# hoyso48/AudioTokenization

Hardware: AMD Instinct MI355X
Metric: audio-sec encoded/sec/GPU (24 kHz mono, 10 s clips) + VQ index bit-exactness (higher is better)
Workload: dtype f32-emulated (x6: 3xbf16, 24-bit operands); 1 GPU; config2: batch=64 x 10 s 24 kHz clips per GPU, encode+VQ (extract_indices path), BigCodec 'default' model, random weights; global_batch=64, clip_samples=240000, parallelism=dp1

## Files before the change

### audiotokenization_amd/csrc/conv1d_x6_kernel.h

```cpp
#pragma once
#include <type_traits>

#include "bc_common.h"
#include "bc_internal.h"
#include "conv_epilogue.h"
#include "x6_common.h"

namespace bc {

struct X6NoMid {};

template <int MT, int NT, int WM, int WN, int P, bool PW, int TPS = 1, bool DB = false, bool B4 = false>
__global__ void __launch_bounds__(64 * WM * WN, (WM * WN == 16 ? 1 : (NT == 1 ? 4 : 2))) conv1d_x6_kernel(ConvArgs a) {
  constexpr int BM = 16 * MT * WM;
  constexpr int BN = 16 * NT * WN;
  constexpr int QA = WM * MT;
  constexpr int NW = WM * WN;
  static_assert(NW == 8 || NW == 16, "512- or 1024-thread workgroups");
  constexpr int NCG = NW / 8;
  constexpr int CI = ((PW ? BN / 32 : X6_MAXCOL_ITERS) + NCG - 1) / NCG;
  constexpr int NQI = 4 * NW;
  constexpr int IT4 = PW ? (BN / 4 + NQI - 1) / NQI : ((32 * X6_MAXCOL_ITERS + 6) / 4 + NQI - 1) / NQI;
  constexpr int NBL = B4 ? 2 * IT4 : 2 * CI;
  extern __shared__ __attribute__((aligned(16))) unsigned char smem_x6[];
// ... 811 lines not shown
          compute(step & 1, 0, tp, mid);
        } else {
          if (step + 1 < nsteps && !BC_ABL(a.dbg, 1)) issue_a(step + 1, (step + 1) & 1);
          if (tp == 0 && c + 1 < a.nchunks && !BC_ABL(a.dbg, 2)) {
            dma_issue_order();
            stage_load(c + 1);
          }
          if (prio) __builtin_amdgcn_s_setprio(1);
#pragma unroll
          for (int tt = 0; tt < TPS; ++tt) {
            const int tap = tp * TPS + tt;
            if (TPS == 1 || tap < K) compute(step & 1, tt, tap, nomid);
          }
        }
        if (prio) __builtin_amdgcn_s_setprio(0);
        if constexpr (DB) {
          if (c + 1 < a.nchunks) {
            if (P == 2 && tp == 1) stage_max((c + 1) & 1);
            if (tp == DB_STORE) {
              if constexpr (P == 2) {
                const float sn = bmax_scale((c + 1) & 1);
                xn = sn < xs ? sn : xs;
              }
              if (!BC_ABL(a.dbg, 4)) stage_store(Bs + ((c + 1) & 1) * P * bplane, xn, c + 1);
            }
          }
        } else if (tp == kst - 1 && c + 1 < a.nchunks) {
          if constexpr (P == 2) stage_max((c + 1) & 1);
          lds_barrier();
          if constexpr (P == 2) h3_next_scale((c + 1) & 1);
          if (!BC_ABL(a.dbg, 4)) stage_store(Bs, xs, c + 1);
        }
        if (tp == 0 && kst > 1 && c + 1 < a.nchunks)
          wait_vmcnt<NBL>();
        else
          asm volatile("s_waitcnt vmcnt(0)" ::: "memory");
        lds_barrier();
      }
      if constexpr (DB && P == 2) rescale_to(xn);
    }
  }

  fin(acc, b, m0, n0, wm, wn, lane, xs);
}

inline constexpr X6Tile kX6Tiles[] = {
    {4, 4, 2, 4},
    {4, 2, 2, 4},
    {4, 2, 4, 2},
    {2, 2, 4, 2},
    {6, 2, 1, 8},
    {4, 2, 1, 8},
    {3, 2, 1, 8},
    {2, 2, 1, 8},
    {1, 2, 1, 8},
    {6, 1, 1, 8},
    {4, 1, 1, 8},
    {3, 1, 1, 8},
    {2, 1, 1, 8},
    {1, 1, 1, 8},
    {6, 2, 2, 4},
    {6, 1, 2, 4},
    {3, 1, 2, 4},
    {4, 1, 2, 4},
    {8, 2, 2, 4},
    {4, 4, 4, 2},
    {6, 4, 2, 4},
    {8, 4, 2, 4},
    {6, 2, 2, 8},
    {3, 2, 2, 4},
    {3, 4, 1, 8},
};
constexpr int X6_NT = sizeof(kX6Tiles) / sizeof(kX6Tiles[0]);

inline size_t x6_lds(const X6Tile& t, int ncol, int planes, int s, int tps = 1, int bbufs = 1) {
  const size_t bplane = (size_t)((ncol * x6_pitch(s) + 15) / 16 * 16);
  return bbufs * planes * bplane + 2 * tps * planes * (size_t)t.WM * t.MT * 1024;
}

inline int x6_tps() {
  static const int v = [] {
    const char* e = getenv("BC_X6_TPS");
    return e && atoi(e) == 1 ? 1 : 2;
  }();
  return v;
}

inline bool x6_pw_on() {
  static const bool v = [] {
    const char* e = getenv("BC_X6_PW");
    return !e || atoi(e) != 0;
  }();
  return v;
}

inline bool x6_db_on() {
  static const bool v = [] {
    const char* e = getenv("BC_X6_DB");
    return !e || atoi(e) != 0;
  }();
  return v;
}

inline bool x6_tps4_on() {
  static const bool v = [] {
    const char* e = getenv("BC_X6_TPS4");
    return !e || atoi(e) != 0;
  }();
  return v;
}

inline bool x6_b4_on() {
  static const bool v = [] {
    const char* e = getenv("BC_X6_B4");
    return !e || atoi(e) != 0;
  }();
  return v;
}

struct X6Variant {
  bool pw;
  int tps;
  bool db;
  size_t lds;
  bool b4;
};
inline X6Variant x6_variant_base(const X6Tile& t, int P, int K, int s, int d) {
  const int ncol = x6_ncol(t, K, s, d);
  const size_t budget = t.NT > 1 ? 160 * 1024 : 80 * 1024;
  auto fits = [&](int tps, int bb) { return x6_lds(t, ncol, P, s, tps, bb) <= budget; };
  if (K == 1 && ncol == x6_BN(t) && x6_pw_on()) return {true, 1, false, x6_lds(t, ncol, P, s), false};
  const int min_kst = P == 2 ? 3 : 2;
  const bool db = x6_db_on() && P <= 2 && t.NT > 1;
  const bool tps2 = P <= 2 && K > 1 && x6_tps() == 2;
  if (P == 1 && t.WM * t.WN == 16 && db && tps2 && x6_tps4_on() && (K + 3) / 4 >= min_kst && fits(4, 2))
    return {false, 4, true, x6_lds(t, ncol, P, s, 4, 2), false};
  if (db && tps2 && (K + 1) / 2 >= min_kst && fits(2, 2)) return {false, 2, true, x6_lds(t, ncol, P, s, 2, 2), false};
  if (tps2 && fits(2, 1)) return {false, 2, false, x6_lds(t, ncol, P, s, 2), false};
  if (db && K >= min_kst && fits(1, 2)) return {false, 1, true, x6_lds(t, ncol, P, s, 1, 2), false};
  return {false, 1, false, x6_lds(t, ncol, P, s), false};
}
inline X6Variant x6_variant(const X6Tile& t, int P, int K, int s, int d, int ps = 0) {
  X6Variant v = x6_variant_base(t, P, K, s, d);
  const bool pw_tile = t.WM * t.WN == 16 || (t.MT == 6 && t.NT == 2 && t.WM == 2 && t.WN == 4);
  v.b4 = s == 1 && ps == 0 && x6_b4_on() && (v.pw ? pw_tile : t.WM * t.WN == 16);
  return v;
}
inline int x6_prio() {
  static const int v = [] {
    const char* e = getenv("BC_X6_PRIO");
    return e ? atoi(e) : 0;
  }();
  return v;
}
inline bool x6_b4_fits(const ConvArgs& a) {
  return a.ps == 0 && a.s == 1 && a.Tin % 4 == 0 && a.xbs % 4 == 0 && ((unsigned long long)a.x & 15) == 0;
}

template <int MT, int NT, int WM, int WN, int P>
static int launch_x6(ConvArgs& a, int B, hipStream_t st) {
  constexpr int BM = 16 * MT * WM, BN = 16 * NT * WN, NTHR = 64 * WM * WN;
  const X6Tile t{MT, NT, WM, WN};
  const int ncol = x6_ncol(t, a.K, a.s, a.d);
  if (ncol > 32 * X6_MAXCOL_ITERS) return BC_ERR_UNSUPPORTED;
  a.ntm = (a.Cout + BM - 1) / BM;
  a.ntn = (a.Nout + BN - 1) / BN;
  a.nchunks = (a.Cin + X6_BKC - 1) / X6_BKC;
  a.win = ncol;
  a.bpitch = x6_pitch(a.s);
  a.bstage = (ncol * a.bpitch + 15) / 16 * 16;
  const long long nwg = (long long)a.ntm * a.ntn * B;
  if (nwg <= 0) return BC_OK;
  if (nwg > 0x7fffffffLL) return BC_ERR_ARG;
  if ((long long)(a.ps ? a.cin0 : a.Cin) * a.Tin * 4 > 0x7fffffffLL) return BC_ERR_UNSUPPORTED;
  a.nwg = (int)nwg;
  a.wsc = P == 2 ? reinterpret_cast<const float*>(reinterpret_cast<const unsigned char*>(a.w) +
                                                  (long long)a.ntm * a.nchunks * a.K * P * t.WM * t.MT * 1024)
                 : nullptr;
  const size_t lds = x6_lds(t, ncol, P, a.s);
  if (lds > 160 * 1024) return BC_ERR_UNSUPPORTED;
  const X6Variant v = x6_variant(t, P, a.K, a.s, a.d, a.ps);
  a.prio = x6_prio();
  constexpr int T2 = P <= 2 ? 2 : 1;
  constexpr bool D2 = P <= 2;
  if constexpr (WM * WN == 16) {
    if (v.b4 && x6_b4_fits(a)) {
      constexpr int T4 = P == 1 ? 4 : P == 2 ? 2 : 1;
      constexpr bool D4 = P == 1;
      if (!v.pw && v.tps == T4 && v.db == D4) {
        hipLaunchKernelGGL((conv1d_x6_kernel<MT, NT, WM, WN, P, false, T4, D4, true>), dim3(a.nwg), dim3(NTHR), v.lds,
                           st, a);
        BC_CHECK_LAUNCH();
        return BC_OK;
      }
    }
  }
  if constexpr (P == 1 && WM * WN == 16) {
    if (v.tps == 4) {
      hipLaunchKernelGGL((conv1d_x6_kernel<MT, NT, WM, WN, P, false, 4, true>), dim3(a.nwg), dim3(NTHR), v.lds, st, a);
      BC_CHECK_LAUNCH();
      return BC_OK;
    }
  }
  if constexpr (WM * WN == 16 || (MT == 6 && NT == 2 && WM == 2 && WN == 4)) {
    if (v.pw && v.b4 && x6_b4_fits(a)) {
      hipLaunchKernelGGL((conv1d_x6_kernel<MT, NT, WM, WN, P, true, 1, false, true>), dim3(a.nwg), dim3(NTHR), v.lds, st, a);
      BC_CHECK_LAUNCH();
      return BC_OK;
    }
  }
  if (v.pw)
    hipLaunchKernelGGL((conv1d_x6_kernel<MT, NT, WM, WN, P, true>), dim3(a.nwg), dim3(NTHR), v.lds, st, a);
  else if (v.db && v.tps == 2)
    hipLaunchKernelGGL((conv1d_x6_kernel<MT, NT, WM, WN, P, false, T2, D2>), dim3(a.nwg), dim3(NTHR), v.lds, st, a);
  else if (v.db)
    hipLaunchKernelGGL((conv1d_x6_kernel<MT, NT, WM, WN, P, false, 1, D2>), dim3(a.nwg), dim3(NTHR), v.lds, st, a);
  else if (v.tps == 2)
    hipLaunchKernelGGL((conv1d_x6_kernel<MT, NT, WM, WN, P, false, T2>), dim3(a.nwg), dim3(NTHR), v.lds, st, a);
  else
    hipLaunchKernelGGL((conv1d_x6_kernel<MT, NT, WM, WN, P, false>), dim3(a.nwg), dim3(NTHR), v.lds, st, a);
  BC_CHECK_LAUNCH();
  return BC_OK;
}

template <int P>
static int launch_x6_w16(ConvArgs& a, int B, hipStream_t st) {
  return launch_x6<6, 2, 2, 8, P>(a, B, st);
}

template <int P>
int x6_launch_tile(ConvArgs& a, int B, int tile, hipStream_t st);

#define BC_X6_TILE_SWITCH(P)                                       \
  switch (tile) {                                                  \
    case 0: return launch_x6<4, 4, 2, 4, P>(a, B, st);             \
    case 1: return launch_x6<4, 2, 2, 4, P>(a, B, st);             \
    case 2: return launch_x6<4, 2, 4, 2, P>(a, B, st);             \
    case 3: return launch_x6<2, 2, 4, 2, P>(a, B, st);             \
    case 4: return launch_x6<6, 2, 1, 8, P>(a, B, st);             \
    case 5: return launch_x6<4, 2, 1, 8, P>(a, B, st);             \
    case 6: return launch_x6<3, 2, 1, 8, P>(a, B, st);             \
    case 7: return launch_x6<2, 2, 1, 8, P>(a, B, st);             \
    case 8: return launch_x6<1, 2, 1, 8, P>(a, B, st);             \
    case 9: return launch_x6<6, 1, 1, 8, P>(a, B, st);             \
    case 10: return launch_x6<4, 1, 1, 8, P>(a, B, st);            \
    case 11: return launch_x6<3, 1, 1, 8, P>(a, B, st);            \
    case 12: return launch_x6<2, 1, 1, 8, P>(a, B, st);            \
    case 13: return launch_x6<1, 1, 1, 8, P>(a, B, st);            \
    case 14: return launch_x6<6, 2, 2, 4, P>(a, B, st);            \
    case 15: return launch_x6<6, 1, 2, 4, P>(a, B, st);            \
    case 16: return launch_x6<3, 1, 2, 4, P>(a, B, st);            \
    case 17: return launch_x6<4, 1, 2, 4, P>(a, B, st);            \
    case 18: return launch_x6<8, 2, 2, 4, P>(a, B, st);            \
    case 19: return launch_x6<4, 4, 4, 2, P>(a, B, st);            \
    case 20: return launch_x6<6, 4, 2, 4, P>(a, B, st);            \
    case 21: return launch_x6<8, 4, 2, 4, P>(a, B, st);            \
    case 22: return launch_x6_w16<P>(a, B, st);                    \
    case 23:                                                       \
    case 24: return BC_ERR_UNSUPPORTED;                            \
  }                                                                \
  return BC_ERR_ARG;

}
```

### audiotokenization_amd/csrc/resunit_x6.hip

```cpp
#include <cstdio>
#include <cstdlib>

#include "bc_common.h"
#include "bc_internal.h"
#include "conv_epilogue.h"
#include "x6_common.h"

namespace bc {

constexpr int RU_MAX_DIL = 9;

struct RUExtra {
  const float* w1;
  const float* s2a;
  const float* s2b;
  int hplane;
  int nck1;
  int dbg;
  const float* isa;
  const float* isb;
};

__device__ __forceinline__ int hs_off(int n, int g) { return n * 64 + 16 * (g ^ ((n >> 2) & 3)); }

constexpr int ru_min_waves(int MT, int NT, int WM, int P) {
  return (NT == 1 || (MT == 3 && NT == 2 && WM == 2)) ? 4 : 2;
}
constexpr int ru_launch_waves(int MT, int NT, int WM, int WN, int P) {
  return WM * WN == 16 ? 1 : ru_min_waves(MT, NT, WM, P);
}
constexpr int ru_npw(int NW, int QA, int NTT) {
  int n = NW / QA < NTT ? NW / QA : NTT;
  while (n > 1 && NTT % n) --n;
  return n;
}

template <int MT, int NT, int WM, int WN, int P, int TPS = 1>
__global__ void __launch_bounds__(64 * WM * WN, ru_launch_waves(MT, NT, WM, WN, P)) resunit_x6_kernel(ConvArgs a, ConvArgs e, RUExtra r) {
  static_assert(P >= 1 && P <= 3, "bf16, h3 or x6 operands");
  typedef typename FragType<P>::type frag_t;
  constexpr int NW = WM * WN;
  static_assert(NW == 8 || NW == 16, "512- or 1024-thread workgroups");
  constexpr int NTHR = 64 * NW;
  constexpr int NCG = NW / 8;
  __shared__ unsigned smax[2][NW];
  constexpr int BN = 16 * NT * WN;
  constexpr int QA = WM * MT;
  constexpr int CI = ((BN + 6 * RU_MAX_DIL + 31) / 32 + NCG - 1) / NCG;
  constexpr int NTT = NT * WN;
  static_assert(QA <= NW, "one m-tile per wave in phase 2");
  constexpr int NPW = ru_npw(NW, QA, NTT);
  constexpr int NTW = NTT / NPW;
  static_assert(NTT % NPW == 0, "n-tile groups");
  constexpr int KC1 = (16 * QA + X6_BKC - 1) / X6_BKC;
  extern __shared__ __attribute__((aligned(16))) unsigned char smem_ru[];

  const int ncol = a.win;
  const int bplane = a.bstage;
  unsigned char* Bs = smem_ru;
  unsigned char* As = smem_ru + P * bplane;
  auto bgrp = [](int col, int g) { return col * 64 + 16 * (g ^ ((col >> 1) & 3)); };
  unsigned char* Hs = smem_ru;

  const int wg = xcd_remap(blockIdx.x, a.nwg);
  const int nt_idx = wg % a.ntn;
  const int b = wg / a.ntn;
  const int n0 = nt_idx * BN;

  const int tid = threadIdx.x;
  const int lane = tid & 63;
  const int wave = __builtin_amdgcn_readfirstlane(tid >> 6);
  const int wm = wave % WM;
  const int wn = wave / WM;

  const unsigned long long xb_u = (unsigned long long)(a.x + (long long)b * a.xbs);
  const unsigned xb_lo = __builtin_amdgcn_readfirstlane((unsigned)xb_u);
  const unsigned xb_hi = __builtin_amdgcn_readfirstlane((unsigned)(xb_u >> 32));
  const int xbytes = __builtin_amdgcn_readfirstlane(a.Cin * a.Tin * 4);
  const __amdgpu_buffer_rsrc_t xr = __builtin_amdgcn_make_buffer_rsrc(
      (void*)(((unsigned long long)xb_hi << 32) | xb_lo), 0, xbytes, 0x00020000);
  const int in0 = n0 - a.pl;

  const int K = a.K;
  const int kst = (K + TPS - 1) / TPS;
  const int nsteps = a.nchunks * kst;
  const int a_pieces = P * QA;

  auto issue_a = [&](const float* w, int step, int buf) {
    const int c = step / kst, t0 = (step - c * kst) * TPS;
    const int n = (K - t0 < TPS ? K - t0 : TPS) * a_pieces;
    const unsigned char* src = reinterpret_cast<const unsigned char*>(w) + (long long)(c * K + t0) * (a_pieces * 1024);
    unsigned char* dst = As + buf * (TPS * a_pieces * 1024);
    if (!BC_DOK(c < a.nchunks && t0 * a_pieces + n <= K * a_pieces)) return;
    for (int q = wave; q < n; q += NW)
      __builtin_amdgcn_global_load_lds((const void*)(src + q * 1024 + lane * 16), (lds_void_t)(dst + q * 1024),
                                       16, 0, 0);
  };

  const int bp = (tid >> 5) & 15;
  const int bcl = tid & 31;
  const int bcg = tid >> 9;
  auto bcol = [&](int i) { return bcl + 32 * (i * NCG + bcg); };
  float bv0[CI], bv1[CI];
  auto load_b = [&](int chunk) {
    const int ci0 = chunk * X6_BKC + 2 * bp;
#pragma unroll
    for (int i = 0; i < CI; ++i) {
      const int col = bcol(i);
      const int ti = in0 + col;
      const bool tin = col < ncol && ti >= 0 && ti < a.Tin;
      const unsigned o0 = (tin && ci0 < a.Cin) ? (unsigned)((ci0 * a.Tin + ti) * 4) : 0xfffffff0u;
      const unsigned o1 = (tin && ci0 + 1 < a.Cin) ? (unsigned)(((ci0 + 1) * a.Tin + ti) * 4) : 0xfffffff0u;
      bv0[i] = __uint_as_float(__builtin_amdgcn_raw_buffer_load_b32(xr, o0, 0, 0));
      bv1[i] = __uint_as_float(__builtin_amdgcn_raw_buffer_load_b32(xr, o1, 0, 0));
    }
  };
  auto bmax_publish = [&](int par) {
    unsigned m = 0;
#pragma unroll
    for (int i = 0; i < CI; ++i) {
      const unsigned u0 = __float_as_uint(fabsf(bv0[i])), u1 = __float_as_uint(fabsf(bv1[i]));
      m = m > u0 ? m : u0;
      m = m > u1 ? m : u1;
    }
    m = wave_max_u32(m);
    if (lane == 0) smax[par][wave] = m;
  };
  auto bmax_scale = [&](int par) {
    unsigned m = smax[par][0];
#pragma unroll
    for (int w = 1; w < NW; ++w) m = m > smax[par][w] ? m : smax[par][w];
    return h3_scale_from_bits(__builtin_amdgcn_readfirstlane(m));
  };
  float xs = 1.f;
  auto activate_b = [&](int chunk) {
    if (!r.isa || BC_ABL(r.dbg, 16)) return;
    const int ci0 = chunk * X6_BKC + 2 * bp;
    const float a0 = ci0 < a.Cin ? r.isa[ci0] : 0.f, b0 = ci0 < a.Cin ? r.isb[ci0] : 0.f;
    const float a1 = ci0 + 1 < a.Cin ? r.isa[ci0 + 1] : 0.f, b1 = ci0 + 1 < a.Cin ? r.isb[ci0 + 1] : 0.f;
#pragma unroll
    for (int i = 0; i < CI; ++i) {
      const f32x2 v = snake_pk((f32x2){bv0[i], bv1[i]}, (f32x2){a0, a1}, (f32x2){b0, b1});
      bv0[i] = v.x;
      bv1[i] = v.y;
    }
  };
  auto store_b = [&]() {
#pragma unroll
    for (int i = 0; i < CI; ++i) {
      const int col = bcol(i);
      if (col < ncol) {
        if constexpr (P == 2) {
          unsigned h, m;
          split2_h(bv0[i] * xs, bv1[i] * xs, h, m);
          unsigned char* p = Bs + bgrp(col, bp >> 2) + (bp & 3) * 4;
          *reinterpret_cast<unsigned*>(p) = h;
          *reinterpret_cast<unsigned*>(p + bplane) = m;
          continue;
        }
        if constexpr (P == 1) {
          *reinterpret_cast<unsigned*>(Bs + bgrp(col, bp >> 2) + (bp & 3) * 4) = pk_bf16(bv0[i], bv1[i]);
          continue;
        }
        unsigned h, m, l;
        split2(bv0[i], bv1[i], h, m, l);
        unsigned char* p = Bs + bgrp(col, bp >> 2) + (bp & 3) * 4;
        *reinterpret_cast<unsigned*>(p) = h;
        *reinterpret_cast<unsigned*>(p + bplane) = m;
        *reinterpret_cast<unsigned*>(p + 2 * bplane) = l;
      }
    }
  };

  floatx4 acc[MT][NT];
#pragma unroll
  for (int i = 0; i < MT; ++i)
#pragma unroll
    for (int j = 0; j < NT; ++j) acc[i][j] = floatx4{0.f, 0.f, 0.f, 0.f};

  const int col_lane = wn * NT * 16 + (lane & 15);

  auto h3_next_scale = [&](int par) {
    const float sn = bmax_scale(par);
    if (sn < xs) {
      const float rr = sn / xs;
#pragma unroll
      for (int i = 0; i < MT; ++i)
#pragma unroll
        for (int j = 0; j < NT; ++j) acc[i][j] *= rr;
      xs = sn;
    }
  };

  issue_a(a.w, 0, 0);
  load_b(0);
  activate_b(0);
  if constexpr (P == 2) {
    bmax_publish(0);
    lds_barrier();
    xs = bmax_scale(0);
  }
  store_b();
  asm volatile("s_waitcnt vmcnt(0)" ::: "memory");
  __syncthreads();


  const bool p2 = wave < QA * NPW;
  const int mq = wave % QA, jg = wave / QA;

  for (int c = 0; c < a.nchunks; ++c) {
    for (int tp = 0; tp < kst; ++tp) {
      const int step = c * kst + tp;
      if (step + 1 < nsteps && !BC_ABL(r.dbg, 1)) issue_a(a.w, step + 1, (step + 1) & 1);
      if (tp == 0 && c + 1 < a.nchunks && !BC_ABL(r.dbg, 2)) {
        dma_issue_order();
        load_b(c + 1);
      }
#pragma unroll
      for (int tt = 0; tt < TPS; ++tt) {
      const int tap = tp * TPS + tt;
      if (TPS > 1 && tap >= K) break;
      if (BC_ABL(r.dbg, 32)) break;
      const unsigned char* Ab = As + (step & 1) * (TPS * a_pieces * 1024) + tt * (a_pieces * 1024);
      const unsigned char* Bcol = Bs + bgrp(col_lane + tap * a.d, lane >> 4);
      frag_t bf[NT][P];
#pragma unroll
      for (int j = 0; j < NT; ++j)
#pragma unroll
        for (int p = 0; p < P; ++p)
          bf[j][p] = *reinterpret_cast<const frag_t*>(Bcol + j * 16 * 64 + p * bplane);
#pragma unroll
      for (int i = 0; i < MT; ++i) {
        const unsigned char* Aq = Ab + (wm * MT + i) * 1024 + lane * 16;
        const frag_t a0 = *reinterpret_cast<const frag_t*>(Aq);
        if constexpr (P == 2) {
          const frag_t a1 = *reinterpret_cast<const frag_t*>(Aq + QA * 1024);
#pragma unroll
          for (int j = 0; j < NT; ++j) {
            floatx4 t = acc[i][j];
            t = __builtin_amdgcn_mfma_f32_16x16x32_f16(a1, bf[j][0], t, 0, 0, 0);
            t = __builtin_amdgcn_mfma_f32_16x16x32_f16(a0, bf[j][1], t, 0, 0, 0);
            t = __builtin_amdgcn_mfma_f32_16x16x32_f16(a0, bf[j][0], t, 0, 0, 0);
            acc[i][j] = t;
          }
          continue;
        } else if constexpr (P == 1) {
#pragma unroll
          for (int j = 0; j < NT; ++j) acc[i][j] = __builtin_amdgcn_mfma_f32_16x16x32_bf16(a0, bf[j][0], acc[i][j], 0, 0, 0);
        } else {
        const bf16x8_t a1 = *reinterpret_cast<const bf16x8_t*>(Aq + QA * 1024);
        const bf16x8_t a2 = *reinterpret_cast<const bf16x8_t*>(Aq + 2 * QA * 1024);
#pragma unroll
        for (int j = 0; j < NT; ++j) {
          floatx4 t = acc[i][j];
          t = __builtin_amdgcn_mfma_f32_16x16x32_bf16(a2, bf[j][0], t, 0, 0, 0);
          t = __builtin_amdgcn_mfma_f32_16x16x32_bf16(a1, bf[j][1], t, 0, 0, 0);
          t = __builtin_amdgcn_mfma_f32_16x16x32_bf16(a0, bf[j][2], t, 0, 0, 0);
          t = __builtin_amdgcn_mfma_f32_16x16x32_bf16(a1, bf[j][0], t, 0, 0, 0);
          t = __builtin_amdgcn_mfma_f32_16x16x32_bf16(a0, bf[j][1], t, 0, 0, 0);
          t = __builtin_amdgcn_mfma_f32_16x16x32_bf16(a0, bf[j][0], t, 0, 0, 0);
          acc[i][j] = t;
        }
        }
      }
      }
      if (tp == kst - 1 && c + 1 < a.nchunks) {
        activate_b(c + 1);
        if constexpr (P == 2) bmax_publish((c + 1) & 1);
        lds_barrier();
        if constexpr (P == 2) h3_next_scale((c + 1) & 1);
        store_b();
      }
      if (tp == 0 && kst > 1 && c + 1 < a.nchunks)
        wait_vmcnt<2 * CI>();
      else
        asm volatile("s_waitcnt vmcnt(0)" ::: "memory");
      lds_barrier();
    }
  }

  frag_t w1f[KC1][P];
#pragma unroll
  for (int kc = 0; kc < KC1; ++kc)
#pragma unroll
    for (int p = 0; p < P; ++p)
      w1f[kc][p] = (p2 && kc < r.nck1 && BC_DOK(mq < QA))
                       ? *reinterpret_cast<const frag_t*>(reinterpret_cast<const unsigned char*>(r.w1) +
                                                          ((kc * P + p) * QA + mq) * 1024 + lane * 16)
                       : frag_t{};
  const int C = a.Cout;
  if (C < r.nck1 * X6_BKC) {
    const int g0 = (C % X6_BKC) / 8;
    for (int idx = tid; idx < P * BN * 4; idx += NTHR) {
      const int p = idx / (BN * 4), n = (idx / 4) % BN, g = idx % 4;
      if (g >= g0)
        *reinterpret_cast<floatx4*>(Hs + p * r.hplane + (r.nck1 - 1) * (BN * 64) + hs_off(n, g)) =
            floatx4{0.f, 0.f, 0.f, 0.f};
    }
  }
  float hs = 1.f;
  if constexpr (P == 2) {
    const float xinv = 1.f / xs;
    unsigned m = 0;
#pragma unroll
    for (int i = 0; i < MT; ++i) {
      const int co = wm * MT * 16 + i * 16 + (lane >> 4) * 4;
      if (co >= C) continue;
#pragma unroll
      for (int pr = 0; pr < 2; ++pr) {
        const int c0 = co + 2 * pr;
        const f32x2 bias = a.bias ? (f32x2){a.bias[c0], a.bias[c0 + 1]} : (f32x2){0.f, 0.f};
        const f32x2 sc = {a.wsc[c0] * xinv, a.wsc[c0 + 1] * xinv};
        const f32x2 sa = {r.s2a[c0], r.s2a[c0 + 1]}, sb = {r.s2b[c0], r.s2b[c0 + 1]};
#pragma unroll
        for (int j = 0; j < NT; ++j) {
          const f32x2 pre = (f32x2){acc[i][j][2 * pr], acc[i][j][2 * pr + 1]} * sc + bias;
          const f32x2 v = BC_ABL(r.dbg, 64) ? pre : snake_pk(pre, sa, sb);
          acc[i][j][2 * pr] = v.x;
          acc[i][j][2 * pr + 1] = v.y;
          const unsigned u0 = __float_as_uint(fabsf(v.x)), u1 = __float_as_uint(fabsf(v.y));
          m = m > u0 ? m : u0;
          m = m > u1 ? m : u1;
        }
      }
    }
    m = wave_max_u32(m);
    if (lane == 0) smax[0][wave] = m;
    lds_barrier();
    hs = bmax_scale(0);
  }
#pragma unroll
  for (int i = 0; i < MT; ++i) {
    const int co = wm * MT * 16 + i * 16 + (lane >> 4) * 4;
    if (co >= C) continue;
    if constexpr (P == 2) {
      unsigned char* hrow = Hs + (co / X6_BKC) * (BN * 64) + (co % 8) * 2;
      const int g = (co % X6_BKC) / 8;
#pragma unroll
      for (int j = 0; j < NT; ++j) {
        const int n = wn * NT * 16 + j * 16 + (lane & 15);
        unsigned h0, m0, h1, m1;
        split2_h(acc[i][j][0] * hs, acc[i][j][1] * hs, h0, m0);
        split2_h(acc[i][j][2] * hs, acc[i][j][3] * hs, h1, m1);
        unsigned char* dst = hrow + hs_off(n, g);
        *reinterpret_cast<u32x2_t*>(dst) = (u32x2_t){h0, h1};
        *reinterpret_cast<u32x2_t*>(dst + r.hplane) = (u32x2_t){m0, m1};
      }
      continue;
    }
    float bias[4], sa[4], sb[4];
#pragma unroll
    for (int q = 0; q < 4; ++q) {
      bias[q] = a.bias ? a.bias[co + q] : 0.f;
      sa[q] = r.s2a[co + q];
      sb[q] = r.s2b[co + q];
    }
    unsigned char* hrow = Hs + (co / X6_BKC) * (BN * 64) + (co % 8) * 2;
    const int g = (co % X6_BKC) / 8;
#pragma unroll
    for (int j = 0; j < NT; ++j) {
      const int n = wn * NT * 16 + j * 16 + (lane & 15);
      float v[4];
      const f32x2 lo = snake_pk((f32x2){acc[i][j][0] + bias[0], acc[i][j][1] + bias[1]}, (f32x2){sa[0], sa[1]},
                                (f32x2){sb[0], sb[1]});
      const f32x2 hi = snake_pk((f32x2){acc[i][j][2] + bias[2], acc[i][j][3] + bias[3]}, (f32x2){sa[2], sa[3]},
                                (f32x2){sb[2], sb[3]});
      v[0] = lo.x, v[1] = lo.y, v[2] = hi.x, v[3] = hi.y;
      if constexpr (P == 1) {
        *reinterpret_cast<u32x2_t*>(hrow + hs_off(n, g)) = (u32x2_t){pk_bf16(v[0], v[1]), pk_bf16(v[2], v[3])};
        continue;
      }
      unsigned h0, m0, l0, h1, m1, l1;
      split2(v[0], v[1], h0, m0, l0);
      split2(v[2], v[3], h1, m1, l1);
      unsigned char* dst = hrow + hs_off(n, g);
      *reinterpret_cast<u32x2_t*>(dst) = (u32x2_t){h0, h1};
      *reinterpret_cast<u32x2_t*>(dst + r.hplane) = (u32x2_t){m0, m1};
      *reinterpret_cast<u32x2_t*>(dst + 2 * r.hplane) = (u32x2_t){l0, l1};
    }
  }
  floatx4 rpre[NTW];
  {
    const float* rb = e.res ? e.res + (long long)b * e.rbs : nullptr;
    const int co = mq * 16 + (lane & 15);
#pragma unroll
    for (int j = 0; j < NTW; ++j) {
      const int nb = n0 + (jg * NTW + j) * 16 + (lane >> 4) * 4;
      rpre[j] = floatx4{0.f, 0.f, 0.f, 0.f};
      if (p2 && rb && e.vec && co < e.Cout && nb + 3 < e.Nout &&
          BC_DOK((long long)co * e.yT + e.ooff + nb + 3 < e.rbs))
        rpre[j] = *reinterpret_cast<const floatx4*>(rb + (long long)co * e.yT + e.ooff + nb);
    }
  }
  lds_barrier();

  if (p2 && !BC_ABL(r.dbg, 8)) {
    floatx4 acc2[1][NTW];
#pragma unroll
    for (int j = 0; j < NTW; ++j) acc2[0][j] = floatx4{0.f, 0.f, 0.f, 0.f};
#pragma unroll
    for (int j = 0; j < NTW; ++j) {
      const int n = (jg * NTW + j) * 16 + (lane & 15);
#pragma unroll
      for (int kc = 0; kc < KC1; ++kc) {
        if (kc >= r.nck1) break;
        const unsigned char* src = Hs + kc * (BN * 64) + hs_off(n, lane >> 4);
        frag_t bf[P];
#pragma unroll
        for (int p = 0; p < P; ++p) bf[p] = *reinterpret_cast<const frag_t*>(src + p * r.hplane);
        floatx4 t = acc2[0][j];
        if constexpr (P == 2) {
          t = __builtin_amdgcn_mfma_f32_16x16x32_f16(bf[0], w1f[kc][1], t, 0, 0, 0);
          t = __builtin_amdgcn_mfma_f32_16x16x32_f16(bf[1], w1f[kc][0], t, 0, 0, 0);
          t = __builtin_amdgcn_mfma_f32_16x16x32_f16(bf[0], w1f[kc][0], t, 0, 0, 0);
          acc2[0][j] = t;
          continue;
        } else if constexpr (P == 1) {
          acc2[0][j] = __builtin_amdgcn_mfma_f32_16x16x32_bf16(bf[0], w1f[kc][0], t, 0, 0, 0);
        } else {
        t = __builtin_amdgcn_mfma_f32_16x16x32_bf16(bf[0], w1f[kc][2], t, 0, 0, 0);
        t = __builtin_amdgcn_mfma_f32_16x16x32_bf16(bf[1], w1f[kc][1], t, 0, 0, 0);
        t = __builtin_amdgcn_mfma_f32_16x16x32_bf16(bf[2], w1f[kc][0], t, 0, 0, 0);
        t = __builtin_amdgcn_mfma_f32_16x16x32_bf16(bf[0], w1f[kc][1], t, 0, 0, 0);
        t = __builtin_amdgcn_mfma_f32_16x16x32_bf16(bf[1], w1f[kc][0], t, 0, 0, 0);
        t = __builtin_amdgcn_mfma_f32_16x16x32_bf16(bf[0], w1f[kc][0], t, 0, 0, 0);
        acc2[0][j] = t;
        }
      }
    }
    if (BC_ABL(r.dbg, 4)) {
      if (acc2[0][0][0] == 1234.5f) e.y[0] = 0.f;
    } else {
      conv_epilogue_res<NTW, P == 2>(e, acc2, b, mq * 16, n0 + jg * NTW * 16, lane, 1.f / hs, rpre);
    }
  }
}

static const int kRUCandidates[] = {109, 111, 110, 116, 112, 113, 117, 106, 104, 105, 123, 124};
static const int kRUCandidatesP12[] = {123, 109, 111, 110, 116, 112, 113, 117, 106, 104, 105, 124};
constexpr size_t RU_LDS_MAX = 80 * 1024;
static size_t ru_lds_budget(const X6Tile& t) { return t.WM * t.WN == 16 ? 160 * 1024 : RU_LDS_MAX; }
static int ru_forced_cfg() {
  static const int v = [] {
    const char* e = getenv("BC_RU_CFG");
    return e ? atoi(e) : 0;
  }();
  return v;
}

static size_t ru_lds(const X6Tile& t, int C, int d, int P, int* bplane, int* hplane, int tps = 1) {
  const int ncol = x6_ncol(t, 7, 1, d);
  *bplane = (ncol * 64 + 15) / 16 * 16;
  *hplane = (C + X6_BKC - 1) / X6_BKC * x6_BN(t) * 64;
  const size_t ph1 = P * (size_t)*bplane + 2 * tps * P * (size_t)t.WM * t.MT * 1024;
  const size_t ph2 = P * (size_t)*hplane;
  return ph1 > ph2 ? ph1 : ph2;
}

static int ru_tps(const X6Tile& t, int C, int d, int P) {
  static const int forced = [] {
    const char* e = getenv("BC_RU_TPS");
    return e ? atoi(e) : 0;
  }();
  int bp, hp;
  if (P == 3) {
    const bool t48 = t.MT == 3 && t.NT == 1 && t.WM == 1;
    return t48 && C <= 64 && forced != 1 && forced != 4 && ru_lds(t, C, d, P, &bp, &hp, 2) <= ru_lds_budget(t) ? 2 : 1;
  }
  if (forced == 1 || forced == 2 || forced == 4) return forced;
  for (int tps : {4, 2})
    if ((tps < 4 || C <= 64) && ru_lds(t, C, d, P, &bp, &hp, tps) <= ru_lds_budget(t)) return tps;
  return 1;
}

int resunit_select_cfg(int C, int d, int mode) {
  if (mode < 1 || mode > 3 || C < 16 || C % 16 || d <= 0) return -1;
  const int P = mode == 3 ? 2 : mode == 2 ? 1 : 3;
  const int forced = ru_forced_cfg();
  if (!forced && resunit_w16_ok(C, d, P)) return P == 1 ? 222 : 122;
  for (int cfg : (P == 3 ? kRUCandidates : kRUCandidatesP12)) {
    const X6Tile& t = x6_tile(cfg);
    if (x6_BM(t) != C) continue;
    if (d > RU_MAX_DIL) return -1;
    int bp, hp;
    const size_t lds = ru_lds(t, C, d, P, &bp, &hp);
    if (forced ? (cfg != forced || lds > 160 * 1024) : lds > ru_lds_budget(t)) continue;
    return cfg + (P == 2 ? 200 : P == 1 ? 100 : 0);
  }
  return -1;
}

bool resunit_cfg_ok(int cfg, int C, int d) {
  const int mode = cfg / 100;
  if (mode < 1 || mode > 3 || C < 16 || C % 16 || d <= 0 || d > RU_MAX_DIL) return false;
  if (cfg == resunit_select_cfg(C, d, mode)) return true;
  const int base = cfg % 100 + 100;
  bool cand = false;
  for (int c : kRUCandidates) cand = cand || c == base;
  if (!cand) return false;
  const X6Tile& t = x6_tile(base);
  const int P = mode == 3 ? 2 : mode == 2 ? 1 : 3;
  int bp, hp;
  return x6_BM(t) == C && ru_lds(t, C, d, P, &bp, &hp, ru_tps(t, C, d, P)) <= 160 * 1024;
}

template <int MT, int NT, int WM, int WN, int P>
static int launch_ru(ConvArgs& a, ConvArgs& e, RUExtra& r, int B, hipStream_t st) {
  constexpr int BN = 16 * NT * WN, NTHR = 64 * WM * WN;
  const X6Tile t{MT, NT, WM, WN};
  int bplane, hplane;
  const int tps = ru_tps(t, a.Cout, a.d, P);
  const size_t lds = ru_lds(t, a.Cout, a.d, P, &bplane, &hplane, tps);
  if (lds > 160 * 1024) return BC_ERR_UNSUPPORTED;
  a.win = x6_ncol(t, 7, 1, a.d);
  a.bstage = bplane;
  a.nchunks = (a.Cin + X6_BKC - 1) / X6_BKC;
  a.ntm = 1;
  a.ntn = (a.Nout + BN - 1) / BN;
  r.hplane = hplane;
  r.nck1 = (a.Cout + X6_BKC - 1) / X6_BKC;
  const long long nwg = (long long)a.ntn * B;
  if (nwg <= 0) return BC_OK;
  if (nwg > 0x7fffffffLL) return BC_ERR_ARG;
  if ((long long)a.Cin * a.Tin * 4 > 0x7fffffffLL) return BC_ERR_UNSUPPORTED;
  a.nwg = (int)nwg;
  if (P == 2) {
    constexpr int QA = MT * WM;
    a.wsc = reinterpret_cast<const float*>(reinterpret_cast<const unsigned char*>(a.w) +
                                           (long long)a.nchunks * 7 * P * QA * 1024);
    e.wsc = reinterpret_cast<const float*>(reinterpret_cast<const unsigned char*>(r.w1) +
                                           (long long)r.nck1 * P * QA * 1024);
  }
  if (P != 3 && tps == 4)
    hipLaunchKernelGGL((resunit_x6_kernel<MT, NT, WM, WN, P, (P != 3 ? 4 : 1)>), dim3(a.nwg), dim3(NTHR), lds, st, a, e, r);
  else if (tps == 2 && (P != 3 || (MT == 3 && NT == 1 && WM == 1)))
    hipLaunchKernelGGL((resunit_x6_kernel<MT, NT, WM, WN, P, (P != 3 || (MT == 3 && NT == 1 && WM == 1) ? 2 : 1)>),
                       dim3(a.nwg), dim3(NTHR), lds, st, a, e, r);
  else
    hipLaunchKernelGGL((resunit_x6_kernel<MT, NT, WM, WN, P>), dim3(a.nwg), dim3(NTHR), lds, st, a, e, r);
  BC_CHECK_LAUNCH();
  return BC_OK;
}

int resunit_kernel_name(int cfg, int C, int d, char* buf, int n) {
  const int mode = cfg / 100;
  if (mode < 1 || mode > 3 || !resunit_cfg_ok(cfg, C, d)) return -1;
  if (cfg == 122 || cfg == 222) {
    const char* e = getenv("BIGCODEC_RU_SNAKE_IN");
    return snprintf(buf, n, "resunit_w16_kernel<%d, %d, true>", cfg == 122 ? 3 : 1, e && atoi(e) == 0 ? 0 : 2);
  }
  if (mode == 3 && resunit_rr_ok(C, d)) return resunit_rr_kernel_name(C, d, buf, n);
  const X6Tile& t = x6_tile(cfg);
  const int P = mode == 3 ? 2 : mode == 2 ? 1 : 3;
  return snprintf(buf, n, "resunit_x6_kernel<%d, %d, %d, %d, %d, %d>", t.MT, t.NT, t.WM, t.WN, P,
                  ru_tps(t, C, d, P));
}

int resunit_launch(const float* x_raw, const float* x_act, const float* w7, const float* b7, const float* s2a,
                   const float* s2b, const float* w1, const float* b1, const float* osa, const float* osb,
                   float* y, float* y2, int B, int C, int T, int d, int pl, int cfg, hipStream_t st,
                   const float* isa, const float* isb) {
  if (cfg >= 300 && cfg < 400 && resunit_rr_ok(C, d)) {
    const int rc = resunit_rr_launch(x_raw, x_act, w7, b7, s2a, s2b, w1, b1, osa, osb, y, y2, B, C, T, d, pl, st,
                                     isa, isb);
    if (rc != BC_ERR_UNSUPPORTED) return rc;
  }
  ConvArgs a{};
  a.x = x_act; a.w = w7; a.bias = b7;
  a.xbs = (long long)C * T;
  a.Cin = C; a.Tin = T; a.Cout = C; a.Nout = T;
  a.K = 7; a.s = 1; a.d = d; a.pl = pl;
  ConvArgs e{};
  e.bias = b1; e.res = x_raw; e.osa = osa; e.osb = osb; e.y = y; e.y2 = y2;
  e.ybs = (long long)C * T; e.rbs = e.ybs;
  e.Cout = C; e.Nout = T; e.yT = T; e.ostride = 1; e.ooff = 0; e.epi = 0;
  e.vec = conv_epilogue_vec_ok(e);
  static const int dbg = [] {
    const char* v = getenv("BC_RU_DEBUG");
    return v ? atoi(v) : 0;
  }();
  RUExtra r{w1, s2a, s2b, 0, 0, dbg, isa, isb};
  if (isa) a.x = x_raw;
  if (cfg == 122 || cfg == 222) {
    const int P = cfg == 122 ? 3 : 1;
    if (!resunit_w16_ok(C, d, P)) return BC_ERR_UNSUPPORTED;
    a.isa = isa;
    a.isb = isb;
    return resunit_w16_launch(a, e, w1, s2a, s2b, B, P, st);
  }
#define BC_RU_CASES(ID, MT, NT, WM, WN)                           \
  case 100 + ID: return launch_ru<MT, NT, WM, WN, 3>(a, e, r, B, st); \
  case 200 + ID: return launch_ru<MT, NT, WM, WN, 1>(a, e, r, B, st); \
  case 300 + ID: return launch_ru<MT, NT, WM, WN, 2>(a, e, r, B, st);
  switch (cfg) {
    BC_RU_CASES(11, 3, 1, 1, 8)
    BC_RU_CASES(10, 4, 1, 1, 8)
    BC_RU_CASES(16, 3, 1, 2, 4)
    BC_RU_CASES(12, 2, 1, 1, 8)
    BC_RU_CASES(13, 1, 1, 1, 8)
    BC_RU_CASES(9, 6, 1, 1, 8)
    BC_RU_CASES(6, 3, 2, 1, 8)
    BC_RU_CASES(4, 6, 2, 1, 8)
    BC_RU_CASES(5, 4, 2, 1, 8)
    BC_RU_CASES(17, 4, 1, 2, 4)
    BC_RU_CASES(23, 3, 2, 2, 4)
    BC_RU_CASES(24, 3, 4, 1, 8)
  }
#undef BC_RU_CASES
  return BC_ERR_ARG;
}

}

BC_DEBUG_EXPORT(resunit_x6)
```

### audiotokenization_amd/csrc/x6_common.h

```cpp
#pragma once
#include <cstddef>

#include "bc_common.h"
#include "bc_internal.h"

namespace bc {

typedef __bf16 bf16x8_t __attribute__((ext_vector_type(8)));
typedef __bf16 bf16x2_t __attribute__((ext_vector_type(2)));
typedef float float2_t __attribute__((ext_vector_type(2)));
typedef unsigned u32x2_t __attribute__((ext_vector_type(2)));
typedef __attribute__((address_space(3))) void* lds_void_t;
typedef _Float16 f16x8_t __attribute__((ext_vector_type(8)));
typedef _Float16 f16x2_t __attribute__((ext_vector_type(2)));

constexpr int X6_BKC = 32;
constexpr int X6_PITCH = 80;
inline int x6_pitch(int s) { return s == 1 ? 64 : 80; }
constexpr int X6_MAXCOL_ITERS = 11;

template <int N>
__device__ __forceinline__ void wait_vmcnt() {
  static_assert(N >= 0 && N < 64, "vmcnt is 6 bits");
  __builtin_amdgcn_s_waitcnt((N & 15) | ((N >> 4) << 14) | (7 << 4) | (15 << 8));
}

__device__ __forceinline__ void dma_issue_order() {
  asm volatile("" ::: "memory");
  __builtin_amdgcn_sched_barrier(0);
}

__device__ __forceinline__ unsigned pk_bf16(float a, float b) {
  const bf16x2_t v = __builtin_convertvector((float2_t){a, b}, bf16x2_t);
  return __builtin_bit_cast(unsigned, v);
}
__device__ __forceinline__ float bf_lo(unsigned p) { return __uint_as_float(p << 16); }
__device__ __forceinline__ float bf_hi(unsigned p) { return __uint_as_float(p & 0xffff0000u); }

__device__ __forceinline__ void split2(float v0, float v1, unsigned& h, unsigned& m, unsigned& l) {
  h = pk_bf16(v0, v1);
  const float r0 = v0 - bf_lo(h), r1 = v1 - bf_hi(h);
  m = pk_bf16(r0, r1);
  const float s0 = r0 - bf_lo(m), s1 = r1 - bf_hi(m);
  l = pk_bf16(s0, s1);
}

__device__ __forceinline__ unsigned pk_f16(float a, float b) {
  const f16x2_t v = __builtin_convertvector((float2_t){a, b}, f16x2_t);
  return __builtin_bit_cast(unsigned, v);
}
__device__ __forceinline__ float f16_lo(unsigned p) {
  return (float)__builtin_bit_cast(f16x2_t, p)[0];
}
__device__ __forceinline__ float f16_hi(unsigned p) {
  return (float)__builtin_bit_cast(f16x2_t, p)[1];
}
__device__ __forceinline__ void split2_h(float v0, float v1, unsigned& h, unsigned& m) {
  h = pk_f16(v0, v1);
  m = pk_f16(v0 - f16_lo(h), v1 - f16_hi(h));
}
__device__ __forceinline__ float h3_scale_from_bits(unsigned amax_bits) {
  int e = (int)(amax_bits >> 23) - 127;
  if (amax_bits == 0) e = 14;
  e = e < -112 ? -112 : (e > 140 ? 140 : e);
  return __uint_as_float((unsigned)(127 + 14 - e) << 23);
}
__device__ __forceinline__ unsigned wave_max_u32(unsigned v) {
#pragma unroll
  for (int o = 32; o >= 1; o >>= 1) {
    const unsigned w = (unsigned)__shfl_xor((int)v, o, 64);
    v = v > w ? v : w;
  }
  return v;
}

template <int P> struct FragType { typedef bf16x8_t type; };
template <> struct FragType<2> { typedef f16x8_t type; };

struct X6Tile {
  int MT, NT, WM, WN;
};
inline int x6_BM(const X6Tile& t) { return 16 * t.MT * t.WM; }
inline int x6_BN(const X6Tile& t) { return 16 * t.NT * t.WN; }
inline int x6_ncol(const X6Tile& t, int K, int s, int d) { return (x6_BN(t) - 1) * s + (K - 1) * d + 1; }
const X6Tile& x6_tile(int cfg);

}
```

Baseline: 2684 audio-sec/s.

## Add 128-bit quad input staging to fused resunit x6 kernel

Adds a B4 variant of the fused residual-unit kernel that loads input activations with 128-bit buffer loads, four time steps per lane, plus 64-bit tail loads for the halo. K is fixed at 7 and the channel-chunk count is derived from the tile height. Odd tile heights get a half-chunk path that zero-fills the unused rows. The aim is to cut the number of global load instructions and their latency in the staging phase, at the cost of a more complex staging path limited to specific tiles and aligned inputs. It is on by default and can be turned off with an env var, and debug hooks are exported.

```diff
diff --git a/audiotokenization_amd/csrc/conv1d_x6_kernel.h b/audiotokenization_amd/csrc/conv1d_x6_kernel.h
--- a/audiotokenization_amd/csrc/conv1d_x6_kernel.h
+++ b/audiotokenization_amd/csrc/conv1d_x6_kernel.h
@@ -987,9 +987,6 @@
     return e ? atoi(e) : 0;
   }();
   return v;
-}
-inline bool x6_b4_fits(const ConvArgs& a) {
-  return a.ps == 0 && a.s == 1 && a.Tin % 4 == 0 && a.xbs % 4 == 0 && ((unsigned long long)a.x & 15) == 0;
 }
 
 template <int MT, int NT, int WM, int WN, int P>
diff --git a/audiotokenization_amd/csrc/resunit_x6.hip b/audiotokenization_amd/csrc/resunit_x6.hip
--- a/audiotokenization_amd/csrc/resunit_x6.hip
+++ b/audiotokenization_amd/csrc/resunit_x6.hip
@@ -1,5 +1,6 @@
 #include <cstdio>
 #include <cstdlib>
+#include <type_traits>
 
 #include "bc_common.h"
 #include "bc_internal.h"
@@ -35,7 +36,11 @@
   return n;
 }
 
-template <int MT, int NT, int WM, int WN, int P, int TPS = 1>
+constexpr bool ru_b4_tile(int MT, int NT, int WM, int WN, int P) {
+  return P == 3 && NT == 1 && WM == 1 && WN == 8 && (MT == 3 || MT == 6);
+}
+
+template <int MT, int NT, int WM, int WN, int P, int TPS = 1, bool B4 = false>
 __global__ void __launch_bounds__(64 * WM * WN, ru_launch_waves(MT, NT, WM, WN, P)) resunit_x6_kernel(ConvArgs a, ConvArgs e, RUExtra r) {
   static_assert(P >= 1 && P <= 3, "bf16, h3 or x6 operands");
   typedef typename FragType<P>::type frag_t;
@@ -47,6 +52,14 @@
   constexpr int BN = 16 * NT * WN;
   constexpr int QA = WM * MT;
   constexpr int CI = ((BN + 6 * RU_MAX_DIL + 31) / 32 + NCG - 1) / NCG;
+  static_assert(!B4 || P == 3, "quad staging: the x6 units");
+  constexpr int NQI = 4 * NW;
+  constexpr int NQH = 8 * NW;
+  static_assert(!B4 || (4 * NQI == BN && 6 * RU_MAX_DIL + 3 <= 2 * NQI && BN + 6 * RU_MAX_DIL + 3 <= 4 * NQH),
+                "quad staging: the quads cover the tile's width, the tail pairs / the half chunk's quads the halo");
+  constexpr bool HALF = B4 && QA % 2 == 1;
+  constexpr int LASTC = QA / 2;
+  constexpr int NBL = B4 ? (HALF ? 2 : 4) : 2 * CI;
   constexpr int NTT = NT * WN;
   static_assert(QA <= NW, "one m-tile per wave in phase 2");
   constexpr int NPW = ru_npw(NW, QA, NTT);
@@ -81,9 +94,10 @@
       (void*)(((unsigned long long)xb_hi << 32) | xb_lo), 0, xbytes, 0x00020000);
   const int in0 = n0 - a.pl;
 
-  const int K = a.K;
+  const int K = B4 ? 7 : a.K;
   const int kst = (K + TPS - 1) / TPS;
-  const int nsteps = a.nchunks * kst;
+  const int nch = B4 ? (QA + 1) / 2 : a.nchunks;
+  const int nsteps = nch * kst;
   const int a_pieces = P * QA;
 
   auto issue_a = [&](const float* w, int step, int buf) {
@@ -91,7 +105,7 @@
     const int n = (K - t0 < TPS ? K - t0 : TPS) * a_pieces;
     const unsigned char* src = reinterpret_cast<const unsigned char*>(w) + (long long)(c * K + t0) * (a_pieces * 1024);
     unsigned char* dst = As + buf * (TPS * a_pieces * 1024);
-    if (!BC_DOK(c < a.nchunks && t0 * a_pieces + n <= K * a_pieces)) return;
+    if (!BC_DOK(c < nch && t0 * a_pieces + n <= K * a_pieces)) return;
     for (int q = wave; q < n; q += NW)
       __builtin_amdgcn_global_load_lds((const void*)(src + q * 1024 + lane * 16), (lds_void_t)(dst + q * 1024),
                                        16, 0, 0);
@@ -101,11 +115,11 @@
   const int bcl = tid & 31;
   const int bcg = tid >> 9;
   auto bcol = [&](int i) { return bcl + 32 * (i * NCG + bcg); };
-  float bv0[CI], bv1[CI];
-  auto load_b = [&](int chunk) {
+  float bv0[B4 ? 1 : CI], bv1[B4 ? 1 : CI];
+  auto load_b = [&](int chunk) __attribute__((always_inline)) {
     const int ci0 = chunk * X6_BKC + 2 * bp;
 #pragma unroll
-    for (int i = 0; i < CI; ++i) {
+    for (int i = 0; i < (B4 ? 0 : CI); ++i) {
       const int col = bcol(i);
       const int ti = in0 + col;
       const bool tin = col < ncol && ti >= 0 && ti < a.Tin;
@@ -118,7 +132,7 @@
   auto bmax_publish = [&](int par) {
     unsigned m = 0;
 #pragma unroll
-    for (int i = 0; i < CI; ++i) {
+    for (int i = 0; i < (B4 ? 0 : CI); ++i) {
       const unsigned u0 = __float_as_uint(fabsf(bv0[i])), u1 = __float_as_uint(fabsf(bv1[i]));
       m = m > u0 ? m : u0;
       m = m > u1 ? m : u1;
@@ -133,21 +147,21 @@
     return h3_scale_from_bits(__builtin_amdgcn_readfirstlane(m));
   };
   float xs = 1.f;
-  auto activate_b = [&](int chunk) {
+  auto activate_b = [&](int chunk) __attribute__((always_inline)) {
     if (!r.isa || BC_ABL(r.dbg, 16)) return;
     const int ci0 = chunk * X6_BKC + 2 * bp;
     const float a0 = ci0 < a.Cin ? r.isa[ci0] : 0.f, b0 = ci0 < a.Cin ? r.isb[ci0] : 0.f;
     const float a1 = ci0 + 1 < a.Cin ? r.isa[ci0 + 1] : 0.f, b1 = ci0 + 1 < a.Cin ? r.isb[ci0 + 1] : 0.f;
 #pragma unroll
-    for (int i = 0; i < CI; ++i) {
+    for (int i = 0; i < (B4 ? 0 : CI); ++i) {
       const f32x2 v = snake_pk((f32x2){bv0[i], bv1[i]}, (f32x2){a0, a1}, (f32x2){b0, b1});
       bv0[i] = v.x;
       bv1[i] = v.y;
     }
   };
-  auto store_b = [&]() {
-#pragma unroll
-    for (int i = 0; i < CI; ++i) {
+  auto store_b = [&]() __attribute__((always_inline)) {
+#pragma unroll
+    for (int i = 0; i < (B4 ? 0 : CI); ++i) {
       const int col = bcol(i);
       if (col < ncol) {
         if constexpr (P == 2) {
@@ -172,6 +186,117 @@
     }
   };
 
+  const int r4 = in0 & 3;
+  const int tq0 = in0 - r4;
+  const int nq4 = (ncol + r4 + 3) >> 2;
+  const int p4 = 8 * (wave & 1) + (lane & 7), qb4 = 8 * (wave >> 1) + (lane >> 3);
+  const int p4h = lane & 7, qbh = 8 * wave + (lane >> 3);
+  const int ct0 = 4 * NQI - r4 + 2 * qb4;
+  typedef std::integral_constant<bool, false> full_t;
+  typedef std::integral_constant<bool, true> half_t;
+  floatx4 bq0, bq1;
+  float2_t bt0, bt1;
+  const bool live_h = 32 * wave - r4 < ncol;
+  const bool live_t = 4 * NQI - r4 + 16 * (wave >> 1) < ncol;
+  auto load_b4 = [&](int chunk, auto H) __attribute__((always_inline)) {
+    constexpr bool half = decltype(H)::value;
+    const int p = half ? p4h : p4, qb = half ? qbh : qb4;
+    const unsigned rowb = (unsigned)a.Tin * 4;
+    const unsigned cb = (unsigned)(chunk * X6_BKC) * rowb;
+    {
+      const int t = tq0 + 4 * qb;
+      const bool ok = (!half || qb < nq4) && t >= 0 && t < a.Tin;
+      const unsigned o0 = ok ? (unsigned)((2 * p * a.Tin + t) * 4) + cb : 0x80000000u;
+      bq0 = __builtin_bit_cast(floatx4, __builtin_amdgcn_raw_buffer_load_b128(xr, o0, 0, 0));
+      bq1 = __builtin_bit_cast(floatx4, __builtin_amdgcn_raw_buffer_load_b128(xr, o0 + rowb, 0, 0));
+    }
+    if constexpr (!half) {
+      const int t = tq0 + 4 * NQI + 2 * qb4;
+      const bool ok = ct0 < ncol && t >= 0 && t < a.Tin;
+      const unsigned o0 = ok ? (unsigned)((2 * p * a.Tin + t) * 4) + cb : 0x80000000u;
+      bt0 = __builtin_bit_cast(float2_t, __builtin_amdgcn_raw_buffer_load_b64(xr, o0, 0, 0));
+      bt1 = __builtin_bit_cast(float2_t, __builtin_amdgcn_raw_buffer_load_b64(xr, o0 + rowb, 0, 0));
+    }
+  };
+  auto activate_b4 = [&](int chunk, auto H) __attribute__((always_inline)) {
+    constexpr bool half = decltype(H)::value;
+    if (!r.isa || BC_ABL(r.dbg, 16)) return;
+    const int c0 = chunk * X6_BKC + 2 * (half ? p4h : p4);
+    const f32x2 sa = {r.isa[c0], r.isa[c0 + 1]}, sb = {r.isb[c0], r.isb[c0 + 1]};
+    if (!half || live_h) {
+#pragma unroll
+      for (int j = 0; j < 4; ++j) {
+        const f32x2 v = snake_pk((f32x2){bq0[j], bq1[j]}, sa, sb);
+        bq0[j] = v.x;
+        bq1[j] = v.y;
+      }
+    }
+    if (!half && live_t) {
+#pragma unroll
+      for (int j = 0; j < 2; ++j) {
+        const f32x2 v = snake_pk((f32x2){bt0[j], bt1[j]}, sa, sb);
+        bt0[j] = v.x;
+        bt1[j] = v.y;
+      }
+    }
+  };
+  auto store_b4 = [&](auto H) __attribute__((always_inline)) {
+    constexpr bool half = decltype(H)::value;
+    const int p = half ? p4h : p4, qb = half ? qbh : qb4;
+    unsigned char* prow = Bs + (p & 3) * 4;
+    auto put = [&](int col, float v0, float v1) __attribute__((always_inline)) {
+      if (col >= 0 && col < ncol) {
+        unsigned h, m, l;
+        split2(v0, v1, h, m, l);
+        unsigned char* q = prow + bgrp(col, p >> 2);
+        *reinterpret_cast<unsigned*>(q) = h;
+        *reinterpret_cast<unsigned*>(q + bplane) = m;
+        *reinterpret_cast<unsigned*>(q + 2 * bplane) = l;
+      }
+    };
+    if (!half || live_h) {
+#pragma unroll
+      for (int j = 0; j < 4; ++j) put(4 * qb - r4 + j, bq0[j], bq1[j]);
+    }
+    if (!half && live_t) {
+#pragma unroll
+      for (int j = 0; j < 2; ++j) put(ct0 + j, bt0[j], bt1[j]);
+    }
+    if constexpr (half) {
+      for (int idx = tid; idx < 2 * ncol; idx += NTHR) {
+        const int col = idx >> 1;
+        unsigned char* q = Bs + col * 64 + (((col >> 2) & 1) ? 0 : 32) + 16 * (idx & 1);
+#pragma unroll
+        for (int pl = 0; pl < P; ++pl) *reinterpret_cast<floatx4*>(q + pl * bplane) = floatx4{0.f, 0.f, 0.f, 0.f};
+      }
+    }
+  };
+  auto is_half = [&](int chunk) __attribute__((always_inline)) { return HALF && (LASTC == 0 || (LASTC == 1 && chunk > 0) || chunk == LASTC); };
+  auto stage_load = [&](int chunk) __attribute__((always_inline)) {
+    if constexpr (B4) {
+      if (is_half(chunk)) load_b4(chunk, half_t{});
+      else load_b4(chunk, full_t{});
+    } else {
+      load_b(chunk);
+    }
+  };
+  auto stage_activate = [&](int chunk) __attribute__((always_inline)) {
+    if constexpr (B4) {
+      if (is_half(chunk)) activate_b4(chunk, half_t{});
+      else activate_b4(chunk, full_t{});
+    } else {
+      activate_b(chunk);
+    }
+  };
+  auto stage_store = [&](int chunk) __attribute__((always_inline)) {
+    if constexpr (B4) {
+      if (is_half(chunk)) store_b4(half_t{});
+      else store_b4(full_t{});
+    } else {
+      store_b();
+    }
+  };
+
   floatx4 acc[MT][NT];
 #pragma unroll
   for (int i = 0; i < MT; ++i)
@@ -193,14 +318,14 @@
   };
 
   issue_a(a.w, 0, 0);
-  load_b(0);
-  activate_b(0);
+  stage_load(0);
+  stage_activate(0);
   if constexpr (P == 2) {
     bmax_publish(0);
     lds_barrier();
     xs = bmax_scale(0);
   }
-  store_b();
+  stage_store(0);
   asm volatile("s_waitcnt vmcnt(0)" ::: "memory");
   __syncthreads();
 
@@ -208,13 +333,13 @@
   const bool p2 = wave < QA * NPW;
   const int mq = wave % QA, jg = wave / QA;
 
-  for (int c = 0; c < a.nchunks; ++c) {
+  for (int c = 0; c < nch; ++c) {
     for (int tp = 0; tp < kst; ++tp) {
       const int step = c * kst + tp;
       if (step + 1 < nsteps && !BC_ABL(r.dbg, 1)) issue_a(a.w, step + 1, (step + 1) & 1);
-      if (tp == 0 && c + 1 < a.nchunks && !BC_ABL(r.dbg, 2)) {
+      if (tp == 0 && c + 1 < nch && !BC_ABL(r.dbg, 2)) {
         dma_issue_order();
-        load_b(c + 1);
+        stage_load(c + 1);
       }
 #pragma unroll
       for (int tt = 0; tt < TPS; ++tt) {
@@ -264,15 +389,15 @@
         }
       }
       }
-      if (tp == kst - 1 && c + 1 < a.nchunks) {
-        activate_b(c + 1);
+      if (tp == kst - 1 && c + 1 < nch) {
+        stage_activate(c + 1);
         if constexpr (P == 2) bmax_publish((c + 1) & 1);
         lds_barrier();
         if constexpr (P == 2) h3_next_scale((c + 1) & 1);
-        store_b();
-      }
-      if (tp == 0 && kst > 1 && c + 1 < a.nchunks)
-        wait_vmcnt<2 * CI>();
+        stage_store(c + 1);
+      }
+      if (tp == 0 && kst > 1 && c + 1 < nch)
+        wait_vmcnt<NBL>();
       else
         asm volatile("s_waitcnt vmcnt(0)" ::: "memory");
       lds_barrier();
@@ -503,6 +628,12 @@
   int bp, hp;
   return x6_BM(t) == C && ru_lds(t, C, d, P, &bp, &hp, ru_tps(t, C, d, P)) <= 160 * 1024;
 }
+
+static int g_ru_b4 = [] {
+  const char* e = getenv("BC_RU_B4");
+  return e && atoi(e) == 0 ? 0 : 1;
+}();
+static int g_ru_last_b4 = -1;
 
 template <int MT, int NT, int WM, int WN, int P>
 static int launch_ru(ConvArgs& a, ConvArgs& e, RUExtra& r, int B, hipStream_t st) {
@@ -531,6 +662,16 @@
     e.wsc = reinterpret_cast<const float*>(reinterpret_cast<const unsigned char*>(r.w1) +
                                            (long long)r.nck1 * P * QA * 1024);
   }
+  if constexpr (ru_b4_tile(MT, NT, WM, WN, P)) {
+    constexpr int TPS4 = MT == 3 ? 2 : 1;
+    if (g_ru_b4 && tps == TPS4 && a.Cin == 16 * MT * WM && x6_b4_fits(a)) {
+      hipLaunchKernelGGL((resunit_x6_kernel<MT, NT, WM, WN, P, TPS4, true>), dim3(a.nwg), dim3(NTHR), lds, st, a, e, r);
+      BC_CHECK_LAUNCH();
+      g_ru_last_b4 = 1;
+      return BC_OK;
+    }
+  }
+  g_ru_last_b4 = 0;
   if (P != 3 && tps == 4)
     hipLaunchKernelGGL((resunit_x6_kernel<MT, NT, WM, WN, P, (P != 3 ? 4 : 1)>), dim3(a.nwg), dim3(NTHR), lds, st, a, e, r);
   else if (tps == 2 && (P != 3 || (MT == 3 && NT == 1 && WM == 1)))
@@ -612,4 +753,12 @@
 
 }
 
+extern "C" int bc_debug_set_ru_quad_staging(int on) {
+  const int old = bc::g_ru_b4;
+  bc::g_ru_b4 = on ? 1 : 0;
+  return old;
+}
+
+extern "C" int bc_debug_ru_last_staging(void) { return bc::g_ru_last_b4; }
+
 BC_DEBUG_EXPORT(resunit_x6)
diff --git a/audiotokenization_amd/csrc/x6_common.h b/audiotokenization_amd/csrc/x6_common.h
--- a/audiotokenization_amd/csrc/x6_common.h
+++ b/audiotokenization_amd/csrc/x6_common.h
@@ -85,4 +85,8 @@
 inline int x6_ncol(const X6Tile& t, int K, int s, int d) { return (x6_BN(t) - 1) * s + (K - 1) * d + 1; }
 const X6Tile& x6_tile(int cfg);
 
+inline bool x6_b4_fits(const ConvArgs& a) {
+  return a.ps == 0 && a.s == 1 && a.Tin % 4 == 0 && a.xbs % 4 == 0 && ((unsigned long long)a.x & 15) == 0;
 }
+
+}
```

Result: no change. 2693 audio-sec/s (median of 6 runs) (+0.4%).
